# uberkk/ImageCompressionLearnedLiftingandLearnedTreeBasedModels

Measured on AMD Instinct MI355X. Metric: Mpixels/sec (lifting DWT + entropy-model fwd) at 512x512 RGB, higher is better.
Workload: dtype f32 storage, f16x3 arithmetic (3 fp16 MFMA products per fp32 MAC, fp32 accumulate)

## Files before the change

### imagecompressionlearnedliftingandlearnedtreebasedmodels_amd/_lib.py

```python
import ctypes as C
import os

_HERE = os.path.dirname(os.path.abspath(__file__))
LIB_PATH = os.path.join(_HERE, "liblldwt.so")


class LLDWTError(RuntimeError):
    pass


class View(C.Structure):
    _fields_ = [("p", C.c_void_p), ("sz", C.c_int64), ("sy", C.c_int64), ("sx", C.c_int64)]


class LiftOp(C.Structure):
    _fields_ = [("kind", C.c_int32), ("buf_src", C.c_int32), ("buf_din", C.c_int32), ("buf_dout", C.c_int32),
                ("off_src", C.c_int64), ("sz_src", C.c_int64), ("sy_src", C.c_int64), ("sx_src", C.c_int64),
                ("off_din", C.c_int64), ("sz_din", C.c_int64), ("sy_din", C.c_int64), ("sx_din", C.c_int64),
                ("off_dout", C.c_int64), ("sz_dout", C.c_int64), ("sy_dout", C.c_int64), ("sx_dout", C.c_int64),
                ("h", C.c_int32), ("w", C.c_int32), ("vertical", C.c_int32), ("tap", C.c_int32), ("block", C.c_int32),
                ("is_u", C.c_int32), ("sign", C.c_float), ("pad_", C.c_int32), ("saved_off", C.c_int64)]


class ConvDesc(C.Structure):
# ... 39 lines not shown
    "lldwt_train_lift_f16": (_i, []),
    "lldwt_set_precision": (_i, [_i]),
    "lldwt_get_precision": (_i, []),
    "lldwt_set_cdf97_short_levels": (_i, [_i]),
    "lldwt_get_lift_mode": (_i, []),
    "lldwt_pack_pblock": (_i, [_p] * 9 + [_i, _i, _i, _p]),
    "lldwt_pack_pblock_train": (_i, [_p] * 9 + [_i, _i, _i, _p]),
    "lldwt_pack_pblock_seq": (_i, [_p] * 9 + [_i, _i, _i, _p]),
    "lldwt_lift_step_ws_bytes": (_i64, [_i64, _i64, _i64, _i]),
    "lldwt_lift_step": (_i, [View, View, View, _i64, _i64, _i64, _i64, _p, _p, _i, _i, _i, _f, _f, _i, _p, _i64, _p]),
    "lldwt_lifting_ws_bytes": (_i64, [_i64, _i64, _i64, _i]),
    "lldwt_lifting_forward": (_i, [_p, _p, C.POINTER(_p), _i64, _i64, _i64, _i64, _i, _p, _p, _i, _i, _i, _i, _i, _f, _i,
                                   _p, _p, _p, _i64, _p]),
    "lldwt_lifting_inverse": (_i, [_p, C.POINTER(_p), _p, _i64, _i64, _i64, _i64, _i, _p, _p, _i, _i, _i, _i, _f, _i,
                                   _p, _p, _p, _i64, _p]),
    "lldwt_lifting_program": (_i, [C.POINTER(LiftOp), _i, _i64, _i64, _i64, _i, _i, _i, _i, _i, _i, C.POINTER(_i64)]),
    "lldwt_lifting_forward_train": (_i, [_p, _p, C.POINTER(_p), _i64, _i64, _i64, _i64, _i, _p, _p, _i, _i, _i, _i, _i, _f,
                                         _i, _p, _p, _p, _i64, _p, _p]),
    "lldwt_lifting_inverse_train": (_i, [_p, C.POINTER(_p), _p, _i64, _i64, _i64, _i64, _i, _p, _p, _i, _i, _i, _i, _f, _i,
                                         _p, _p, _p, _i64, _p, _p]),
    "lldwt_lift_bwd_pre": (_i, [View, View, _p, _i64, _i64, _i64, _p]),
    "lldwt_lift_bwd_fin": (_i, [_p, _p, _p, View, _i64, _i64, _i64, _i64, _p, _p, _i, _f, _f, _p]),
    "lldwt_lift_step_bwd_ws_bytes": (_i64, [_i64, _i64, _i64, _i]),
    "lldwt_lift_step_bwd": (_i, [View, View, View, _p, _i64, _i64, _i64, _i64, _p, _p, _p, _i64] + [_p] * 8 +
                            [_i, _i, _f, _f, _i, _i, _p, _i64, _p]),
    "lldwt_lift_step_bwd_f16": (_i, [View, View, View, _p, _i64, _i64, _i64, _i64, _p, _p, _p, _i64] + [_p] * 8 +
                                [_i, _i, _f, _f, _i, _i, _p, _i64, _p, _p, _p]),
    "lldwt_bwd_lift_f16": (_i, []),
    "lldwt_pack_pblock_bwd_ws_bytes": (_i64, [_i]),
    "lldwt_pack_pblock_bwd": (_i, [_p, _p, _p, _p, _p, _p, _i64, _i, _i, _i, _p]),
    "lldwt_subband_mlp_bwd_w_ws_bytes": (_i64, [_i64, _i, _i64]),
    "lldwt_subband_mlp_bwd_w": (_i, [_p, _p, _p, _i64, _i64, _i, _i64, _i] + [_p] * 7 + [_p] * 8 + [_p, _i64, _p]),
    "lldwt_subband_mlp_bwd": (_i, [_p] * 9 + [_i64, _i64, _i, _i64, _i] + [_p] * 7 + [_p]),
    "lldwt_subband_mlp": (_i, [_p, _p, _i64, _i64, _i, _i64, _i] + [_p] * 8 + [_i, _p]),
    "lldwt_conv_packed_floats": (_i64, [C.POINTER(ConvDesc)]),
    "lldwt_conv_pack": (_i, [_p, _p, C.POINTER(ConvDesc), _i64, _i, _p]),
    "lldwt_conv2d": (_i, [_p, _p, _p, _p, _p, _p, C.POINTER(ConvDesc), _i64, _i64, _i64, _i64, _p]),
    "lldwt_conv_stack_pair": (_i, [_p, _p, _p, _p, C.POINTER(_p), C.POINTER(_p), C.POINTER(ConvDesc), _i, _i, _p, _p, _i64, _i64, _i64,
                                   _i64, _i64, _i64, _p]),
    "lldwt_conv2d_absmax": (_i, [_p, _p, _p, _p, _p, _p, _p, C.POINTER(ConvDesc), _i64, _i64, _i64, _i64, _p]),
    "lldwt_conv2d_f16out": (_i, [_p, _p, _p, _p, _p, C.POINTER(ConvDesc), _i64, _i64, _i64, _i64, _p]),
    "lldwt_conv3x3_f16in": (_i, [_p, _p, _p, _p, _p, _i, _i, _i, _i64, _i64, _i64, _i64, _p]),
    "lldwt_conv2d_wgrad": (_i, [_p, _p, _p, _p, C.POINTER(ConvDesc), _i64, _i64, _i64, _i64, _f, _i, _p]),
    "lldwt_conv3x3_wgrad_f16x3": (_i, [_p, _p, _p, _p, _p, _p, _p, _i, _i, _i64, _i64, _i64, _i64, _f, _p]),
    "lldwt_conv_f16x3_packed_bytes": (_i64, [_i, _i]),
    "lldwt_plc_shape16": (_i, []),
    "lldwt_plc_winograd": (_i, []),
    "lldwt_plc_fused_pack1_bytes": (_i64, [_i]),
    "lldwt_plc_fused_pack1": (_i, [_p, _p, _p, _i, _i64, _p]),
    "lldwt_plc_fused": (_i, [_p, _p, _p, _p, _p, _i, _i, _i, _i64, _i64, _i64, _i64, _p]),
    "lldwt_conv_f16x3_pack": (_i, [_p, _p, _i, _i, _i64, _p]),
    "lldwt_absmax_slots": (_i, [_p, _i64, _i64, _p, _p]),
    "lldwt_conv3x3_f16x3": (_i, [_p, _p, _p, _p, _p, _i, _i, _i, _i64, _i64, _i64, _i64, _p]),
    "lldwt_act_bwd": (_i, [_p, _p, _p, _i64, _i, _p]),
    "lldwt_downsum2": (_i, [_p, _p, _i64, _i64, _i64, _p]),
    "lldwt_conv2d_direct": (_i, [_p, _p, _p, _p, C.POINTER(ConvDesc), _i64, _i64, _i64, _i64, _p]),
    "lldwt_gdn": (_i, [_p, _p, _p, _p, _i64, _i64, _i, _i64, _i, _f, _p]),
    "lldwt_ew_mul": (_i, [_p, _p, _p, _i64, _f, _p]),
    "lldwt_gdn_apply": (_i, [_p, _p, _p, _i64, _i, _p]),
    "lldwt_gdn_apply_bwd": (_i, [_p, _p, _p, _p, _p, _i64, _i, _p]),
    "lldwt_lower_bound_fwd": (_i, [_p, _p, _i64, _f, _p]),
    "lldwt_lower_bound_bwd": (_i, [_p, _p, _p, _i64, _f, _p]),
    "lldwt_nonneg_param_fwd": (_i, [_p, _p, _i64, _f, _p]),
    "lldwt_nonneg_param_bwd": (_i, [_p, _p, _p, _i64, _f, _p]),
    "lldwt_gauss_rate": (_i, [_p, _p, _p, _p, _p, _p, _i64, _i, _i64, _p]),
    "lldwt_cgp_packed_floats": (_i64, [_i, _i, _i, _i, _i]),
    "lldwt_cgp_pack": (_i, [_p] * 9 + [_i64, _i, _i, _i, _i, _i, _p]),
# ... 89 lines not shown
```

### imagecompressionlearnedliftingandlearnedtreebasedmodels_amd/csrc/ops.hip

```cpp
#include "common.h"
#include <stdlib.h>
#include <string.h>
#include <math.h>

namespace lldwt {

static thread_local char g_err[512] = "";

void set_error(const char* fmt, ...) {
    va_list ap;
    va_start(ap, fmt);
    vsnprintf(g_err, sizeof(g_err), fmt, ap);
    va_end(ap);
}

constexpr float KR = 0.2126f, KG = 0.7152f, KB = 0.0722f;

__global__ void k_rgb_to_ycc(const float* __restrict__ rgb, float* __restrict__ ycc, int64_t B, int64_t hw) {
    const int64_t n = B * hw;
    for (int64_t i = blockIdx.x * (int64_t)blockDim.x + threadIdx.x; i < n; i += (int64_t)gridDim.x * blockDim.x) {
        const int64_t b = i / hw, p = i - b * hw;
        const float r = rgb[(b * 3 + 0) * hw + p], g = rgb[(b * 3 + 1) * hw + p], bl = rgb[(b * 3 + 2) * hw + p];
        const float y = KR * r + KG * g + KB * bl;
        const float cb = 0.5f * (bl - y) / (1.f - KB) + 0.5f;
// ... 144 lines not shown
                                  uint32_t tw, uint32_t ov, uint32_t ny, uint32_t nx, uint32_t y0, uint32_t x0, uint32_t h,
                                  uint32_t w, float inv_ov, float* __restrict__ acc) {
    const uint32_t x = blockIdx.x * blockDim.x + threadIdx.x;
    if (x >= w) return;
    const LapAxis ay = lap_axis(y0 + blockIdx.y, th, ov, ny, inv_ov);
    const LapAxis ax = lap_axis(x0 + x, tw, ov, nx, inv_ov);
    const int32_t qy[2] = {ay.q0, ay.q1}, iy[2] = {ay.i0, ay.i1}, qx[2] = {ax.q0, ax.q1}, ix[2] = {ax.i0, ax.i1};
    const float wy[2] = {ay.w0, ay.w1}, wx[2] = {ax.w0, ax.w1};
    const int64_t hw = (int64_t)th * tw, rhw = (int64_t)h * w, p = (int64_t)blockIdx.y * w + x;
    float a[3];
    bool any = false;
#pragma unroll
    for (int c = 0; c < 3; ++c) a[c] = acc[c * rhw + p];
#pragma unroll
    for (int u = 0; u < 2; ++u) {
#pragma unroll
        for (int v = 0; v < 2; ++v) {
            if (qy[u] < 0 || qx[v] < 0) continue;
            const int32_t j = slots[(int64_t)qy[u] * nx + qx[v]];
            if (j < 0 || j >= n) continue;
            const float wt = __fmul_rn(wy[u], wx[v]);
            const int64_t q = (int64_t)iy[u] * tw + ix[v];
#pragma unroll
            for (int c = 0; c < 3; ++c) a[c] = __fadd_rn(a[c], __fmul_rn(wt, ycc[(c * n + j) * hw + q]));
            any = true;
        }
    }
    if (!any) return;
#pragma unroll
    for (int c = 0; c < 3; ++c) acc[c * rhw + p] = a[c];
}

typedef float floatx4m __attribute__((ext_vector_type(4)));
__global__ __launch_bounds__(256) void k_subband_mlp_mfma(const float* __restrict__ x, float* __restrict__ y, int batch, int C,
                                                          int64_t hw, const float* __restrict__ w0,
                                                          const float* __restrict__ b0, const float* __restrict__ w1,
                                                          const float* __restrict__ b1, const float* __restrict__ w2,
                                                          const float* __restrict__ b2, const float* __restrict__ w3,
                                                          const float* __restrict__ b3, int transposed) {
    constexpr int HD = 32;
    const int c = blockIdx.y;
    const int64_t z = blockIdx.z;
    const int plane = (int)(z / batch);
    const int64_t pc = (int64_t)plane * C + c;
    const int lane = threadIdx.x & 63, wave = threadIdx.x >> 6;
    const int col = lane & 15, kk = lane >> 4;
    float A1[2][8], A2[2][8], w0b[8], b0b[8], b1d[8], b2d[8], w3d[8];
#pragma unroll
    for (int m = 0; m < 2; ++m)
#pragma unroll
        for (int q = 0; q < 8; ++q) {
            const int oc = m * 16 + col, ic = (q >> 2) * 16 + 4 * kk + (q & 3);
            const int64_t src = transposed ? (pc * HD + ic) * HD + oc : (pc * HD + oc) * HD + ic;
            A1[m][q] = w1[src];
            A2[m][q] = w2[src];
        }
#pragma unroll
    for (int q = 0; q < 8; ++q) {
        const int ch = (q >> 2) * 16 + 4 * kk + (q & 3);
        w0b[q] = w0[pc * HD + ch];
        b0b[q] = b0[pc * HD + ch];
        b1d[q] = b1[pc * HD + ch];
        b2d[q] = b2[pc * HD + ch];
        w3d[q] = w3[pc * HD + ch];
    }
    const float bb3 = b3[pc];
    const float* xp = x + (z * C + c) * hw;
    float* yp = y + (z * C + c) * hw;
    for (int64_t i0 = ((int64_t)blockIdx.x * 4 + wave) * 64; i0 < hw; i0 += (int64_t)gridDim.x * 256) {
        float xv[4];
#pragma unroll
        for (int n = 0; n < 4; ++n) {
            const int64_t i = i0 + n * 16 + col;
            xv[n] = xp[i < hw ? i : 0];
        }
        float h[4][8];
#pragma unroll
        for (int n = 0; n < 4; ++n)
#pragma unroll
            for (int q = 0; q < 8; ++q) h[n][q] = fast_tanh(fmaf(w0b[q], xv[n], b0b[q]));
#pragma unroll
        for (int layer = 0; layer < 2; ++layer) {
            floatx4m acc[2][4];
#pragma unroll
            for (int m = 0; m < 2; ++m)
#pragma unroll
                for (int n = 0; n < 4; ++n) {
                    const float* bd = layer == 0 ? b1d : b2d;
                    acc[m][n] = floatx4m{bd[m * 4 + 0], bd[m * 4 + 1], bd[m * 4 + 2], bd[m * 4 + 3]};
                }
#pragma unroll
            for (int q = 0; q < 8; ++q)
#pragma unroll
                for (int m = 0; m < 2; ++m)
#pragma unroll
                    for (int n = 0; n < 4; ++n)
                        acc[m][n] = __builtin_amdgcn_mfma_f32_16x16x4f32(layer == 0 ? A1[m][q] : A2[m][q], h[n][q], acc[m][n],
                                                                         0, 0, 0);
#pragma unroll
            for (int n = 0; n < 4; ++n)
#pragma unroll
                for (int m = 0; m < 2; ++m)
#pragma unroll
                    for (int r = 0; r < 4; ++r) h[n][m * 4 + r] = fast_tanh(acc[m][n][r]);
        }
#pragma unroll
        for (int n = 0; n < 4; ++n) {
            float o = 0.f;
#pragma unroll
            for (int q = 0; q < 8; ++q) o = fmaf(w3d[q], h[n][q], o);
            o += __shfl_xor(o, 16, 64);
            o += __shfl_xor(o, 32, 64);
            const int64_t i = i0 + n * 16 + col;
            if (kk == 0 && i < hw) yp[i] = o + bb3;
        }
    }
}

__global__ __launch_bounds__(256) void k_subband_mlp_bwd(const float* __restrict__ x, const float* __restrict__ gy,
                                                         float* __restrict__ gx, float* __restrict__ h0o,
                                                         float* __restrict__ h1o, float* __restrict__ h2o,
                                                         float* __restrict__ d0o, float* __restrict__ d1o,
                                                         float* __restrict__ d2o, int batch, int C, int64_t hw,
                                                         const float* __restrict__ w0, const float* __restrict__ b0,
                                                         const float* __restrict__ w1, const float* __restrict__ b1,
                                                         const float* __restrict__ w2, const float* __restrict__ b2,
                                                         const float* __restrict__ w3) {
    constexpr int HD = 32, NC = 2;
    const int c = blockIdx.y;
    const int64_t z = blockIdx.z;
    const int plane = (int)(z / batch);
    const int64_t pc = (int64_t)plane * C + c;
    const int lane = threadIdx.x & 63, wave = threadIdx.x >> 6;
    const int col = lane & 15, kk = lane >> 4;
    float A1[2][8], A2[2][8], A1T[2][8], A2T[2][8], w0b[8], b0b[8], b1d[8], b2d[8], w3d[8];
#pragma unroll
    for (int m = 0; m < 2; ++m)
#pragma unroll
        for (int q = 0; q < 8; ++q) {
            const int row = m * 16 + col, ch = (q >> 2) * 16 + 4 * kk + (q & 3);
            A1[m][q] = w1[(pc * HD + row) * HD + ch];
            A2[m][q] = w2[(pc * HD + row) * HD + ch];
            A1T[m][q] = w1[(pc * HD + ch) * HD + row];
            A2T[m][q] = w2[(pc * HD + ch) * HD + row];
        }
#pragma unroll
    for (int q = 0; q < 8; ++q) {
        const int ch = (q >> 2) * 16 + 4 * kk + (q & 3);
        w0b[q] = w0[pc * HD + ch];
        b0b[q] = b0[pc * HD + ch];
// ... 975 lines not shown
    return check_launch("u8hwc_to_ycc_tiles_lapped");
}
extern "C" int lldwt_ycc_tiles_blend(const float* ycc, const int32_t* slots, int64_t nslots, int64_t n, int64_t H, int64_t W,
                                     int64_t th, int64_t tw, int64_t ov, int64_t ny, int64_t nx, int64_t y0, int64_t x0,
                                     int64_t h, int64_t w, float* acc, void* stream) {
    LLDWT_REQUIRE(ycc && slots && acc, "ycc_tiles_blend: null pointer");
    if (const int rc = lapped_grid_ok("ycc_tiles_blend", H, W, th, tw, ov, ny, nx)) return rc;
    LLDWT_REQUIRE(ny * nx < (1ll << 31) && nslots == ny * nx, "ycc_tiles_blend: the slot table holds %lld entries, the grid "
                  "has %lld tiles", (long long)nslots, (long long)(ny * nx));
    LLDWT_REQUIRE(n > 0 && n <= nslots, "ycc_tiles_blend: %lld tiles in the group, the grid has %lld", (long long)n,
                  (long long)nslots);
    LLDWT_REQUIRE(y0 >= 0 && x0 >= 0 && h > 0 && w > 0 && y0 + h <= H && x0 + w <= W,
                  "ycc_tiles_blend: region (%lld, %lld, %lld, %lld) outside the %lld x %lld image", (long long)y0,
                  (long long)x0, (long long)h, (long long)w, (long long)H, (long long)W);
    LLDWT_REQUIRE(h <= 65535, "ycc_tiles_blend: grid too large");
    hipLaunchKernelGGL(k_ycc_tiles_blend, dim3((unsigned)cdiv(w, 256), (unsigned)h), dim3(256), 0, (hipStream_t)stream, ycc,
                       slots, n, (uint32_t)th, (uint32_t)tw, (uint32_t)ov, (uint32_t)ny, (uint32_t)nx, (uint32_t)y0,
                       (uint32_t)x0, (uint32_t)h, (uint32_t)w, 1.0f / (float)ov, acc);
    return check_launch("ycc_tiles_blend");
}
extern "C" int lldwt_u8hwc_to_ycc_pad(const uint8_t* src, float* ycc, int64_t B, int64_t H, int64_t W, int64_t Hp, int64_t Wp,
                                      void* stream) {
    LLDWT_REQUIRE(src && ycc && B > 0 && H > 0 && W > 0 && Hp >= H && Wp >= W, "u8hwc_to_ycc_pad: bad arguments");
    LLDWT_REQUIRE(B <= 65535 && Hp <= 65535 && Wp <= (1ll << 30), "u8hwc_to_ycc_pad: grid too large");
    return lldwt_u8hwc_to_ycc_tiles(src, ycc, B, H, W, Hp, Wp, 1, 1, 0, B, stream);
}
extern "C" int lldwt_ycc_to_u8hwc_crop(const float* ycc, uint8_t* dst, int64_t B, int64_t H, int64_t W, int64_t Hp, int64_t Wp,
                                       void* stream) {
    LLDWT_REQUIRE(ycc && dst && B > 0 && H > 0 && W > 0 && Hp >= H && Wp >= W, "ycc_to_u8hwc_crop: bad arguments");
    LLDWT_REQUIRE(B <= 65535 && H <= 65535 && W <= (1ll << 30), "ycc_to_u8hwc_crop: grid too large");
    return lldwt_ycc_tiles_to_u8hwc(ycc, nullptr, 0, B, B, H, W, Hp, Wp, 1, 1, 0, 0, H, W, dst, stream);
}

extern "C" int lldwt_subband_mlp(const float* x, float* y, int64_t planes, int64_t batch, int C, int64_t hw, int Hd,
                                 const float* w0, const float* b0, const float* w1, const float* b1, const float* w2,
                                 const float* b2, const float* w3, const float* b3, int transposed, void* stream) {
    LLDWT_REQUIRE(x && y && w0 && b0 && w1 && b1 && w2 && b2 && w3 && b3, "subband_mlp: null pointer");
    LLDWT_REQUIRE(planes > 0 && batch > 0 && C > 0 && hw > 0, "subband_mlp: bad dims");
    LLDWT_REQUIRE(Hd == 32, "subband_mlp: hidden width %d unsupported (reference uses H=32, lifting_dwt_nets.py:98)", Hd);
    LLDWT_REQUIRE(planes * batch <= 65535 && C <= 65535, "subband_mlp: grid too large");
    int64_t gx = cdiv(hw, 256);
    if (gx > 1024) gx = 1024;
    dim3 grid((unsigned)gx, (unsigned)C, (unsigned)(planes * batch));
    hipLaunchKernelGGL(k_subband_mlp_mfma, grid, dim3(256), 0, (hipStream_t)stream, x, y, (int)batch, C, hw, w0, b0, w1, b1,
                       w2, b2, w3, b3, transposed);
    return check_launch("subband_mlp");
}

extern "C" int lldwt_subband_mlp_bwd(const float* x, const float* gy, float* gx, float* h0, float* h1, float* h2, float* d0,
                                     float* d1, float* d2, int64_t planes, int64_t batch, int C, int64_t hw, int Hd,
                                     const float* w0, const float* b0, const float* w1, const float* b1, const float* w2,
                                     const float* b2, const float* w3, void* stream) {
    LLDWT_REQUIRE(x && gy && gx && h0 && h1 && h2 && d0 && d1 && d2 && w0 && b0 && w1 && b1 && w2 && b2 && w3,
                  "subband_mlp_bwd: null pointer");
    LLDWT_REQUIRE(planes > 0 && batch > 0 && C > 0 && hw > 0, "subband_mlp_bwd: bad dims");
    LLDWT_REQUIRE(Hd == 32, "subband_mlp_bwd: hidden width %d unsupported (reference uses H=32, lifting_dwt_nets.py:98)", Hd);
    LLDWT_REQUIRE(planes * batch <= 65535 && C <= 65535, "subband_mlp_bwd: grid too large");
    int64_t gxn = cdiv(hw, 128);
    if (gxn > 1024) gxn = 1024;
    dim3 grid((unsigned)gxn, (unsigned)C, (unsigned)(planes * batch));
    hipLaunchKernelGGL(k_subband_mlp_bwd, grid, dim3(256), 0, (hipStream_t)stream, x, gy, gx, h0, h1, h2, d0, d1, d2, (int)batch,
                       C, hw, w0, b0, w1, b1, w2, b2, w3);
    return check_launch("subband_mlp_bwd");
}

static inline int64_t mlpw_slices(int64_t planes, int C, int64_t hw) {
    int64_t s = (int64_t)lldwt_num_cus() * 2 / (planes * C);
    const int64_t most = cdiv(hw, 128);
    s = s > most ? most : s;
    return s < 1 ? 1 : s;
}
extern "C" int64_t lldwt_subband_mlp_bwd_w_ws_bytes(int64_t planes, int C, int64_t hw) {
    return (int64_t)sizeof(float) * planes * C * mlpw_slices(planes, C, hw) * 4 * MLPW_ROW;
}
extern "C" int lldwt_subband_mlp_bwd_w(const float* x, const float* gy, float* gx, int64_t planes, int64_t batch, int C, int64_t hw,
                                       int Hd, const float* w0, const float* b0, const float* w1, const float* b1,
                                       const float* w2, const float* b2, const float* w3, float* dw0, float* db0, float* dw1,
                                       float* db1, float* dw2, float* db2, float* dw3, float* db3, void* ws, int64_t ws_bytes,
                                       void* stream) {
    LLDWT_REQUIRE(x && gy && gx && w0 && b0 && w1 && b1 && w2 && b2 && w3 && dw0 && db0 && dw1 && db1 && dw2 && db2 && dw3 && db3 &&
                  ws, "subband_mlp_bwd_w: null pointer");
// ... 264 lines not shown
```

### imagecompressionlearnedliftingandlearnedtreebasedmodels_amd/graphs/layers/lifting_dwt_nets.py

```python
import torch
from torch import nn

from ... import ops
from ...packed_cache import PackedOwnerMixin, cached
from .P_block_v2 import P_block_v2
from .gdn import GDN
from .wavelet_forward_v2 import wavelet_forward_v2
from .wavelet_inverse_v2 import wavelet_inverse_v2

lifting_coeff = [-1.586134342059924, -0.052980118572961, 0.882911075530934, 0.443506852043971, 0.869864451624781,
                 1.149604398860241]


def get_cdf97_filters(oned_or_twod="2D"):
    lp = torch.tensor([0.0, 0.037828455507264, -0.023849465019557, -0.110624404418437, 0.377402855612831,
                       0.852698679008894, 0.377402855612831, -0.110624404418437, -0.023849465019557,
                       0.037828455507264], dtype=torch.double)
    hp = torch.tensor([0.0, -0.064538882628697, 0.040689417609164, 0.418092273221617, -0.788485616405583,
                       0.418092273221617, 0.040689417609164, -0.064538882628697, 0.0, 0.0], dtype=torch.double)
    slp = torch.tensor([0.0, -0.064538882628697, -0.040689417609164, 0.418092273221617, 0.788485616405583,
                        0.418092273221617, -0.040689417609164, -0.064538882628697, 0.0, 0.0], dtype=torch.double)
    shp = torch.tensor([0.0, -0.037828455507264, -0.023849465019557, 0.110624404418437, 0.377402855612831,
                        -0.852698679008894, 0.377402855612831, 0.110624404418437, -0.023849465019557,
                        -0.037828455507264], dtype=torch.double)
# ... 32 lines not shown


class SubbandAutoEncoderBerk(PackedOwnerMixin, nn.Module):

    def __init__(self, in_ch):
        super().__init__()
        self._init_packed_owner()
        iC, H, K, P = in_ch, 64, 3, 1
        self.in_ch = iC
        self.ae_down = nn.Sequential(
            nn.Conv2d(iC, iC * H // 2, K, padding=P), GDN(iC * H // 2), nn.Conv2d(iC * H // 2, iC * H, K, padding=P),
            GDN(iC * H), nn.Conv2d(iC * H, iC * H // 2, K, padding=P), GDN(iC * H // 2),
            nn.Conv2d(iC * H // 2, iC, K, padding=P))
        self.ae_up = nn.Sequential(
            nn.ConvTranspose2d(iC, iC * H // 2, K, padding=P), GDN(iC * H // 2, inverse=True),
            nn.ConvTranspose2d(iC * H // 2, iC * H, K, padding=P), GDN(iC * H, inverse=True),
            nn.ConvTranspose2d(iC * H, iC * H // 2, K, padding=P), GDN(iC * H // 2, inverse=True),
            nn.ConvTranspose2d(iC * H // 2, iC, K, padding=P))

    def encode(self, x):
        return ae_planes([self], x[None].contiguous(), False)[0]

    def decode(self, y_hat):
        return ae_planes([self], y_hat[None].contiguous(), True)[0]


def ae_planes(aes, x, decode):
    seq = [(a.ae_up if decode else a.ae_down) for a in aes]
    tag = ("ae", decode)
    own = aes[0]
    if isinstance(aes[0], SubbandAutoEncoder):
        convs = [[s[n] for s in seq] for n in (0, 2, 4, 6)]
        srcs = [p for layer in convs for m in layer for p in (m.weight, m.bias)]
        ws = cached(own, tag, srcs, lambda: [t for layer in convs for t in (
            _stack(layer, lambda m: m.weight).flatten(1), _stack(layer, lambda m: m.bias))])
        return ops.subband_mlp(x, *ws, transposed=decode, hidden=aes[0].H)
    t = x
    for n in (0, 2, 4, 6):
        layer = [s[n] for s in seq]
        w, b = cached(own, tag + (n,), [p for m in layer for p in (m.weight, m.bias)],
                          lambda: (_stack(layer, lambda m: m.weight), _stack(layer, lambda m: m.bias)))
        t = ops.conv2d(t, w, b, 3, transposed=decode)
        if n != 6:
            g = [s[n + 1] for s in seq]
            beta, gamma = cached(own, tag + (n, "g"), [p for m in g for p in (m.beta, m.gamma)],
                                     lambda: (_stack(g, lambda m: m.beta), _stack(g, lambda m: m.gamma)))
            t = ops.gdn(t, beta, gamma, inverse=decode, beta_min=g[0].beta_min)
    return t


class DWTPytorchWaveletsLayer(PackedOwnerMixin, nn.Module):

    def __init__(self, config):
        super().__init__()
        self._init_packed_owner()
        self.dwtlevels = config.dwtlevels
        self.clrch = config.clrch
        self.Yl_ae = SubbandAutoEncoder(in_ch=1 * config.clrch)
        self.Yh_ae = nn.ModuleList([SubbandAutoEncoder(in_ch=3 * config.clrch) for _ in range(self.dwtlevels)])

    def encode(self, x):
        xe, xo = encode_planes([self], x[None].contiguous())
        return xe[0], [t[0] for t in xo]

    def decode(self, out_xe, out_xo_list):
        return decode_planes([self], out_xe[None].contiguous(), [t[None].contiguous() for t in out_xo_list])[0]


class LiftingBasedNeuralWaveletv4(PackedOwnerMixin, nn.Module):
# ... 177 lines not shown
```

### imagecompressionlearnedliftingandlearnedtreebasedmodels_amd/ops.py

```python
import ctypes as C
import os

import torch

from . import _lib
from ._lib import (ACT_LRELU, ACT_NONE, ACT_RELU, ACT_TANH, EPI_LRELU_BWD, EPI_NONE, EPI_TANH_BWD, ConvDesc, View,
                   check)

_ws = {}


def _env_choice(name, default, allowed):
    v = os.environ.get(name, default)
    if v not in allowed:
        names = " or ".join(a if a.isdigit() else repr(a) for a in allowed)
        raise _lib.LLDWTError("%s must be %s (got %r)" % (name, names, v))
    return v


def plc_mode():
    return _env_choice("LLDWT_PLC_MODE", "f16x3", ("f32", "f16x3"))


def train_lift_f16():
# ... 333 lines not shown
    check(_lib.load().lldwt_set_cdf97_short_levels(1 if periodic else 0), "lldwt_set_cdf97_short_levels")


def cdf97_forward(x, levels, adj=False):
    lib = _lib.load()
    P, B, Cc, H, W = x.shape
    Z = P * B * Cc
    dev = x.device
    ll = torch.empty(P, B, Cc, H >> levels, W >> levels, device=dev, dtype=torch.float32)
    yh = [torch.empty(P, B, Cc, 3, H >> (i + 1), W >> (i + 1), device=dev, dtype=torch.float32) for i in range(levels)]
    nb = lib.lldwt_cdf97_ws_bytes(Z, H, W)
    ws = workspace(nb, dev)
    check(lib.lldwt_cdf97_forward(_chk(x, "x"), _chk(ll), _ptr_array(yh), Z, H, W, levels, int(bool(adj)),
                                     C.c_void_p(ws.data_ptr()), nb, _stream()), "cdf97_forward")
    return ll, yh


def cdf97_inverse(ll, yh, adj=False):
    lib = _lib.load()
    levels = len(yh)
    P, B, Cc, hl, wl = ll.shape
    H, W = hl << levels, wl << levels
    Z = P * B * Cc
    x = torch.empty(P, B, Cc, H, W, device=ll.device, dtype=torch.float32)
    for t in yh:
        _chk(t, "yh")
    nb = lib.lldwt_cdf97_ws_bytes(Z, H, W)
    ws = workspace(nb, ll.device)
    check(lib.lldwt_cdf97_inverse(_chk(ll, "ll"), _ptr_array(yh), _chk(x), Z, H, W, levels, int(bool(adj)),
                                     C.c_void_p(ws.data_ptr()), nb, _stream()), "cdf97_inverse")
    return x


def subband_mlp(x, w0, b0, w1, b1, w2, b2, w3, b3, transposed=False, hidden=32):
    lib = _lib.load()
    P, B, Cc, h, w = x.shape
    y = torch.empty_like(x)
    check(lib.lldwt_subband_mlp(_chk(x, "x"), _chk(y), P, B, Cc, h * w, hidden, _chk(w0), _chk(b0), _chk(w1), _chk(b1),
                                _chk(w2), _chk(b2), _chk(w3), _chk(b3), int(bool(transposed)), _stream()), "subband_mlp")
    return y


def subband_mlp_bwd(x, gy, w0, b0, w1, b1, w2, b2, w3, hidden=32):
    P, B, Cc, h, w = x.shape
    gx = torch.empty_like(x)
    hs = [torch.empty(P, B, Cc * hidden, h, w, device=x.device, dtype=torch.float32) for _ in range(6)]
    check(_lib.load().lldwt_subband_mlp_bwd(_chk(x, "x"), _chk(gy, "gy"), _chk(gx), *[_chk(t) for t in hs], P, B, Cc, h * w,
                                            hidden, _chk(w0), _chk(b0), _chk(w1), _chk(b1), _chk(w2), _chk(b2), _chk(w3),
                                            _stream()), "subband_mlp_bwd")
    return gx, hs[:3], hs[3:]


def subband_mlp_bwd_w(x, gy, w0, b0, w1, b1, w2, b2, w3, hidden=32):
    lib = _lib.load()
    P, B, Cc, h, w = x.shape
    gx = torch.empty_like(x)
    shapes = [(P, Cc * hidden, 1, 1, 1), (P, Cc * hidden), (P, Cc * hidden, hidden, 1, 1), (P, Cc * hidden),
              (P, Cc * hidden, hidden, 1, 1), (P, Cc * hidden), (P, Cc, hidden, 1, 1), (P, Cc)]
    g = [torch.empty(s, device=x.device, dtype=torch.float32) for s in shapes]
    nb = lib.lldwt_subband_mlp_bwd_w_ws_bytes(P, Cc, h * w)
    ws = workspace(nb, x.device)
    check(lib.lldwt_subband_mlp_bwd_w(_chk(x, "x"), _chk(gy, "gy"), _chk(gx), P, B, Cc, h * w, hidden, _chk(w0), _chk(b0),
                                      _chk(w1), _chk(b1), _chk(w2), _chk(b2), _chk(w3), *[_chk(t) for t in g],
                                      C.c_void_p(ws.data_ptr()), nb, _stream()), "subband_mlp_bwd_w")
    return gx, g


def conv_desc(cin, cout, K, groups=1, act=ACT_NONE, upsample2=False, transposed=False, tap_mask=None, oc_block=None,
              oc_stride=0, oc_off=0, ytot=None, ic_block=0, ic_stride=0, ic_off=0, xtot=0, epi=0):
    return ConvDesc(cin, cout, K, groups, act, int(bool(upsample2)), int(bool(transposed)),
                    (1 << (K * K)) - 1 if tap_mask is None else int(tap_mask), cout if oc_block is None else oc_block,
                    oc_stride, oc_off, cout if ytot is None else ytot, ic_block, ic_stride, ic_off, xtot, epi)
# ... 801 lines not shown
```

### include/lldwt.h

```cpp
#ifndef LLDWT_H
#define LLDWT_H

#include <stdint.h>

#ifdef __cplusplus
extern "C" {
#endif

#define LLDWT_OK 0
#define LLDWT_EINVAL (-1)
#define LLDWT_EHIP (-2)
#define LLDWT_EWS (-3)

#define LLDWT_ACT_NONE 0
#define LLDWT_ACT_TANH 1
#define LLDWT_ACT_LRELU 2
#define LLDWT_ACT_RELU 3

const char* lldwt_last_error(void);
int lldwt_version(void);
int lldwt_device_ok(void);

typedef struct lldwt_view {
    float* p;
// ... 70 lines not shown
                          int block_offset, int inverse, int scale, int C, int64_t* saved_floats);
int lldwt_lifting_forward_train(const float* x, float* ll, float* const* yh, int64_t planes, int64_t batch, int64_t H,
                                int64_t W, int levels, const float* taps, const float* packed, int nblocks,
                                int block_offset, int different, int C, int K, float res_weight, int linear,
                                const float* scale_nh, const float* scale_nl, void* ws, int64_t ws_bytes, float* saved,
                                void* stream);
int lldwt_lifting_inverse_train(const float* ll, const float* const* yh, float* x, int64_t planes, int64_t batch,
                                int64_t H, int64_t W, int levels, const float* taps, const float* packed, int nblocks,
                                int block_offset, int C, int K, float res_weight, int linear, const float* scale_nh,
                                const float* scale_nl, void* ws, int64_t ws_bytes, float* saved, void* stream);
int lldwt_lift_bwd_pre(lldwt_view g_dst_out, lldwt_view g_dst_in, float* g, int64_t Z, int64_t h, int64_t w, void* stream);
int lldwt_lift_bwd_fin(const float* g, const float* dsk, const float* srcv, lldwt_view g_src, int64_t Z, int64_t batch,
                       int64_t h, int64_t w, const float* taps, float* dtaps, int vertical, float sign, float res_weight,
                       void* stream);

int64_t lldwt_lift_step_bwd_ws_bytes(int64_t Z, int64_t h, int64_t w, int C);
int lldwt_lift_step_bwd(lldwt_view g_dst_out, lldwt_view g_dst_in, lldwt_view g_src, const float* saved_step,
                        int64_t planes, int64_t batch, int64_t h, int64_t w, const float* taps, float* dtaps,
                        const float* packed, int64_t packed_plane_stride, float* dw1, float* db1, float* dw2, float* db2,
                        float* dw3, float* db3, float* dw4, float* db4, int C, int K, float res_weight, float sign,
                        int vertical, int linear, void* ws, int64_t ws_bytes, void* stream);

int lldwt_bwd_lift_f16(void);
int64_t lldwt_pack_pblock_bwd_ws_bytes(int planes);
int lldwt_pack_pblock_bwd(const float* w1, const float* w2, const float* w3, const float* w4, float* packed, void* ws,
                          int64_t ws_bytes, int planes, int C, int K, void* stream);
int lldwt_lift_step_bwd_f16(lldwt_view g_dst_out, lldwt_view g_dst_in, lldwt_view g_src, const float* saved_step,
                            int64_t planes, int64_t batch, int64_t h, int64_t w, const float* taps, float* dtaps,
                            const float* packed, int64_t packed_plane_stride, float* dw1, float* db1, float* dw2, float* db2,
                            float* dw3, float* db3, float* dw4, float* db4, int C, int K, float res_weight, float sign,
                            int vertical, int linear, void* ws, int64_t ws_bytes, const float* packed_bwd,
                            const float* taps_id, void* stream);

int lldwt_subband_mlp(const float* x, float* y, int64_t planes, int64_t batch, int C, int64_t hw, int Hd,
                      const float* w0, const float* b0, const float* w1, const float* b1, const float* w2,
                      const float* b2, const float* w3, const float* b3, int transposed, void* stream);
int lldwt_subband_mlp_bwd(const float* x, const float* gy, float* gx, float* h0, float* h1, float* h2, float* d0, float* d1,
                          float* d2, int64_t planes, int64_t batch, int C, int64_t hw, int Hd, const float* w0,
                          const float* b0, const float* w1, const float* b1, const float* w2, const float* b2,
                          const float* w3, void* stream);
int64_t lldwt_subband_mlp_bwd_w_ws_bytes(int64_t planes, int C, int64_t hw);
int lldwt_subband_mlp_bwd_w(const float* x, const float* gy, float* gx, int64_t planes, int64_t batch, int C, int64_t hw, int Hd,
                            const float* w0, const float* b0, const float* w1, const float* b1, const float* w2,
                            const float* b2, const float* w3, float* dw0, float* db0, float* dw1, float* db1, float* dw2,
                            float* db2, float* dw3, float* db3, void* ws, int64_t ws_bytes, void* stream);

typedef struct lldwt_conv_desc {
    int cin, cout, K, groups;
    int act;
    int upsample2;
    int transposed;
    uint32_t tap_mask;
    int oc_block, oc_stride, oc_off, ytot;
    int ic_block, ic_stride, ic_off, xtot;
    int epi;
} lldwt_conv_desc;
#define LLDWT_EPI_NONE 0
#define LLDWT_EPI_TANH_BWD 1
#define LLDWT_EPI_LRELU_BWD 2
int64_t lldwt_conv_packed_floats(const lldwt_conv_desc* d);
int lldwt_conv_pack(const float* w, float* packed, const lldwt_conv_desc* d, int64_t planes, int swap_hw, void* stream);
int lldwt_conv2d(const float* x, float* y, const float* packed, const float* bias, const float* residual,
                 const float* aux, const lldwt_conv_desc* d, int64_t planes, int64_t batch, int64_t h, int64_t w_,
                 void* stream);
int lldwt_conv_stack_pair(const float* xa, const float* xb, float* ya, float* yb, const float* const* packed,
                          const float* const* bias, const lldwt_conv_desc* descs, int nlayers, int groups_a, float* ws0,
                          float* ws1, int64_t ws0_floats, int64_t ws1_floats, int64_t planes, int64_t batch, int64_t h, int64_t w_, void* stream);
int lldwt_conv2d_absmax(const float* x, float* y, const float* packed, const float* bias, const float* residual,
                        const float* aux, float* absmax_slots, const lldwt_conv_desc* d, int64_t planes, int64_t batch,
// ... 191 lines not shown
```

Before: 197.2.

## Move subband MLP to split-fp16 MFMA with prepacked cached weights

```diff
diff --git a/imagecompressionlearnedliftingandlearnedtreebasedmodels_amd/_lib.py b/imagecompressionlearnedliftingandlearnedtreebasedmodels_amd/_lib.py
--- a/imagecompressionlearnedliftingandlearnedtreebasedmodels_amd/_lib.py
+++ b/imagecompressionlearnedliftingandlearnedtreebasedmodels_amd/_lib.py
@@ -95,7 +95,9 @@
     "lldwt_subband_mlp_bwd_w_ws_bytes": (_i64, [_i64, _i, _i64]),
     "lldwt_subband_mlp_bwd_w": (_i, [_p, _p, _p, _i64, _i64, _i, _i64, _i] + [_p] * 7 + [_p] * 8 + [_p, _i64, _p]),
     "lldwt_subband_mlp_bwd": (_i, [_p] * 9 + [_i64, _i64, _i, _i64, _i] + [_p] * 7 + [_p]),
-    "lldwt_subband_mlp": (_i, [_p, _p, _i64, _i64, _i, _i64, _i] + [_p] * 8 + [_i, _p]),
+    "lldwt_subband_mlp_packed_bytes": (_i64, [_i64, _i]),
+    "lldwt_subband_mlp_pack": (_i, [_p] * 8 + [_i64, _i, _i, _i, _p, _i64, _p]),
+    "lldwt_subband_mlp": (_i, [_p, _p, _i64, _i64, _i, _i64, _i, _p, _i64, _p]),
     "lldwt_conv_packed_floats": (_i64, [C.POINTER(ConvDesc)]),
     "lldwt_conv_pack": (_i, [_p, _p, C.POINTER(ConvDesc), _i64, _i, _p]),
     "lldwt_conv2d": (_i, [_p, _p, _p, _p, _p, _p, C.POINTER(ConvDesc), _i64, _i64, _i64, _i64, _p]),
diff --git a/imagecompressionlearnedliftingandlearnedtreebasedmodels_amd/csrc/ops.hip b/imagecompressionlearnedliftingandlearnedtreebasedmodels_amd/csrc/ops.hip
--- a/imagecompressionlearnedliftingandlearnedtreebasedmodels_amd/csrc/ops.hip
+++ b/imagecompressionlearnedliftingandlearnedtreebasedmodels_amd/csrc/ops.hip
@@ -200,90 +200,6 @@
 }
 
 typedef float floatx4m __attribute__((ext_vector_type(4)));
-__global__ __launch_bounds__(256) void k_subband_mlp_mfma(const float* __restrict__ x, float* __restrict__ y, int batch, int C,
-                                                          int64_t hw, const float* __restrict__ w0,
-                                                          const float* __restrict__ b0, const float* __restrict__ w1,
-                                                          const float* __restrict__ b1, const float* __restrict__ w2,
-                                                          const float* __restrict__ b2, const float* __restrict__ w3,
-                                                          const float* __restrict__ b3, int transposed) {
-    constexpr int HD = 32;
-    const int c = blockIdx.y;
-    const int64_t z = blockIdx.z;
-    const int plane = (int)(z / batch);
-    const int64_t pc = (int64_t)plane * C + c;
-    const int lane = threadIdx.x & 63, wave = threadIdx.x >> 6;
-    const int col = lane & 15, kk = lane >> 4;
-    float A1[2][8], A2[2][8], w0b[8], b0b[8], b1d[8], b2d[8], w3d[8];
-#pragma unroll
-    for (int m = 0; m < 2; ++m)
-#pragma unroll
-        for (int q = 0; q < 8; ++q) {
-            const int oc = m * 16 + col, ic = (q >> 2) * 16 + 4 * kk + (q & 3);
-            const int64_t src = transposed ? (pc * HD + ic) * HD + oc : (pc * HD + oc) * HD + ic;
-            A1[m][q] = w1[src];
-            A2[m][q] = w2[src];
-        }
-#pragma unroll
-    for (int q = 0; q < 8; ++q) {
-        const int ch = (q >> 2) * 16 + 4 * kk + (q & 3);
-        w0b[q] = w0[pc * HD + ch];
-        b0b[q] = b0[pc * HD + ch];
-        b1d[q] = b1[pc * HD + ch];
-        b2d[q] = b2[pc * HD + ch];
-        w3d[q] = w3[pc * HD + ch];
-    }
-    const float bb3 = b3[pc];
-    const float* xp = x + (z * C + c) * hw;
-    float* yp = y + (z * C + c) * hw;
-    for (int64_t i0 = ((int64_t)blockIdx.x * 4 + wave) * 64; i0 < hw; i0 += (int64_t)gridDim.x * 256) {
-        float xv[4];
-#pragma unroll
-        for (int n = 0; n < 4; ++n) {
-            const int64_t i = i0 + n * 16 + col;
-            xv[n] = xp[i < hw ? i : 0];
-        }
-        float h[4][8];
-#pragma unroll
-        for (int n = 0; n < 4; ++n)
-#pragma unroll
-            for (int q = 0; q < 8; ++q) h[n][q] = fast_tanh(fmaf(w0b[q], xv[n], b0b[q]));
-#pragma unroll
-        for (int layer = 0; layer < 2; ++layer) {
-            floatx4m acc[2][4];
-#pragma unroll
-            for (int m = 0; m < 2; ++m)
-#pragma unroll
-                for (int n = 0; n < 4; ++n) {
-                    const float* bd = layer == 0 ? b1d : b2d;
-                    acc[m][n] = floatx4m{bd[m * 4 + 0], bd[m * 4 + 1], bd[m * 4 + 2], bd[m * 4 + 3]};
-                }
-#pragma unroll
-            for (int q = 0; q < 8; ++q)
-#pragma unroll
-                for (int m = 0; m < 2; ++m)
-#pragma unroll
-                    for (int n = 0; n < 4; ++n)
-                        acc[m][n] = __builtin_amdgcn_mfma_f32_16x16x4f32(layer == 0 ? A1[m][q] : A2[m][q], h[n][q], acc[m][n],
-                                                                         0, 0, 0);
-#pragma unroll
-            for (int n = 0; n < 4; ++n)
-#pragma unroll
-                for (int m = 0; m < 2; ++m)
-#pragma unroll
-                    for (int r = 0; r < 4; ++r) h[n][m * 4 + r] = fast_tanh(acc[m][n][r]);
-        }
-#pragma unroll
-        for (int n = 0; n < 4; ++n) {
-            float o = 0.f;
-#pragma unroll
-            for (int q = 0; q < 8; ++q) o = fmaf(w3d[q], h[n][q], o);
-            o += __shfl_xor(o, 16, 64);
-            o += __shfl_xor(o, 32, 64);
-            const int64_t i = i0 + n * 16 + col;
-            if (kk == 0 && i < hw) yp[i] = o + bb3;
-        }
-    }
-}
 
 __global__ __launch_bounds__(256) void k_subband_mlp_bwd(const float* __restrict__ x, const float* __restrict__ gy,
                                                          float* __restrict__ gx, float* __restrict__ h0o,
@@ -1325,21 +1241,6 @@
     return lldwt_ycc_tiles_to_u8hwc(ycc, nullptr, 0, B, B, H, W, Hp, Wp, 1, 1, 0, 0, H, W, dst, stream);
 }
 
-extern "C" int lldwt_subband_mlp(const float* x, float* y, int64_t planes, int64_t batch, int C, int64_t hw, int Hd,
-                                 const float* w0, const float* b0, const float* w1, const float* b1, const float* w2,
-                                 const float* b2, const float* w3, const float* b3, int transposed, void* stream) {
-    LLDWT_REQUIRE(x && y && w0 && b0 && w1 && b1 && w2 && b2 && w3 && b3, "subband_mlp: null pointer");
-    LLDWT_REQUIRE(planes > 0 && batch > 0 && C > 0 && hw > 0, "subband_mlp: bad dims");
-    LLDWT_REQUIRE(Hd == 32, "subband_mlp: hidden width %d unsupported (reference uses H=32, lifting_dwt_nets.py:98)", Hd);
-    LLDWT_REQUIRE(planes * batch <= 65535 && C <= 65535, "subband_mlp: grid too large");
-    int64_t gx = cdiv(hw, 256);
-    if (gx > 1024) gx = 1024;
-    dim3 grid((unsigned)gx, (unsigned)C, (unsigned)(planes * batch));
-    hipLaunchKernelGGL(k_subband_mlp_mfma, grid, dim3(256), 0, (hipStream_t)stream, x, y, (int)batch, C, hw, w0, b0, w1, b1,
-                       w2, b2, w3, b3, transposed);
-    return check_launch("subband_mlp");
-}
-
 extern "C" int lldwt_subband_mlp_bwd(const float* x, const float* gy, float* gx, float* h0, float* h1, float* h2, float* d0,
                                      float* d1, float* d2, int64_t planes, int64_t batch, int C, int64_t hw, int Hd,
                                      const float* w0, const float* b0, const float* w1, const float* b1, const float* w2,
diff --git a/imagecompressionlearnedliftingandlearnedtreebasedmodels_amd/csrc/subband_mlp_f16.hip b/imagecompressionlearnedliftingandlearnedtreebasedmodels_amd/csrc/subband_mlp_f16.hip
--- /dev/null
+++ b/imagecompressionlearnedliftingandlearnedtreebasedmodels_amd/csrc/subband_mlp_f16.hip
@@ -0,0 +1,200 @@
+#include "split_f16.h"
+
+namespace lldwt {
+namespace {
+
+constexpr int SMLP_HD = 32;
+constexpr int SMLP_A_FLOATS = 2048, SMLP_V_FLOATS = 160, SMLP_S_FLOATS = 8;
+constexpr int SMLP_PC_FLOATS = SMLP_A_FLOATS + SMLP_V_FLOATS + SMLP_S_FLOATS;
+constexpr float SMLP_ACT_SCALE = 16384.f;
+
+__device__ __forceinline__ int smlp_channel(int kk, int j) { return (j >> 2) * 16 + 4 * kk + (j & 3); }
+
+__global__ __launch_bounds__(64) void k_subband_mlp_pack(const float* __restrict__ w0, const float* __restrict__ b0,
+                                                         const float* __restrict__ w1, const float* __restrict__ b1,
+                                                         const float* __restrict__ w2, const float* __restrict__ b2,
+                                                         const float* __restrict__ w3, const float* __restrict__ b3,
+                                                         int transposed, float* __restrict__ pack) {
+    constexpr int HD = SMLP_HD;
+    const int64_t pc = blockIdx.x;
+    const int lane = threadIdx.x, col = lane & 15, kk = lane >> 4;
+    float* out = pack + pc * SMLP_PC_FLOATS;
+    float scale[2];
+#pragma unroll
+    for (int layer = 0; layer < 2; ++layer) {
+        const float* W = (layer == 0 ? w1 : w2) + pc * HD * HD;
+        float amax = 0.f;
+        for (int i = lane; i < HD * HD; i += 64) amax = fmaxf(amax, fabsf(W[i]));
+#pragma unroll
+        for (int o = 32; o > 0; o >>= 1) amax = fmaxf(amax, __shfl_xor(amax, o, 64));
+        const float s = fminf(fmaxf(pow2_scale<15>(amax), 0x1p-113f), 0x1p112f);
+        scale[layer] = s;
+#pragma unroll
+        for (int m = 0; m < 2; ++m) {
+            float v[8];
+#pragma unroll
+            for (int j = 0; j < 8; ++j) {
+                const int oc = m * 16 + col, ic = smlp_channel(kk, j);
+                v[j] = W[transposed ? ic * HD + oc : oc * HD + ic] * s;
+            }
+            h8_t hi, lo;
+            split8v(v, hi, lo);
+            h8_t* frag = reinterpret_cast<h8_t*>(out) + ((layer * 2 + m) * 2) * 64 + lane;
+            frag[0] = hi;
+            frag[64] = lo;
+        }
+    }
+    if (lane < 32) {
+        const int k4 = lane >> 3, j = lane & 7, ch = smlp_channel(k4, j);
+        const float* src[5] = {w0, b0, b1, b2, w3};
+#pragma unroll
+        for (int a = 0; a < 5; ++a) out[SMLP_A_FLOATS + a * 32 + lane] = src[a][pc * HD + ch];
+    }
+    if (lane < 8) {
+        float v = 0.f;
+        if (lane < 2) v = scale[lane];
+        else if (lane < 4) v = (1.f / scale[lane - 2]) * (1.f / SMLP_ACT_SCALE);
+        else if (lane == 4) v = b3[pc];
+        out[SMLP_A_FLOATS + SMLP_V_FLOATS + lane] = v;
+    }
+}
+
+__device__ __forceinline__ float tanh_act(float x) {
+    const float e = __builtin_amdgcn_exp2f(fabsf(x) * 2.88539008177792681472f);
+    const float t = __builtin_fmaf(-2.f * SMLP_ACT_SCALE, __builtin_amdgcn_rcpf(e + 1.f), SMLP_ACT_SCALE);
+    return copysignf(t, x);
+}
+
+__global__ __launch_bounds__(256, 2) void k_subband_mlp_f16(const float* __restrict__ x, float* __restrict__ y, int batch, int C,
+                                                         int64_t hw, int64_t nblk, const float* __restrict__ pack) {
+    const int64_t pc = blockIdx.y;
+    const int plane = (int)(pc / C), c = (int)(pc % C);
+    const int lane = threadIdx.x & 63, wave = threadIdx.x >> 6;
+    const int col = lane & 15, kk = lane >> 4;
+    const float* pk = pack + pc * SMLP_PC_FLOATS;
+    h8_t A[2][2][2];
+#pragma unroll
+    for (int f = 0; f < 8; ++f) A[f >> 2][(f >> 1) & 1][f & 1] = reinterpret_cast<const h8_t*>(pk)[f * 64 + lane];
+    float vec[5][8];
+#pragma unroll
+    for (int a = 0; a < 5; ++a)
+#pragma unroll
+        for (int hlf = 0; hlf < 2; ++hlf) {
+            const floatx4 v = reinterpret_cast<const floatx4*>(pk + SMLP_A_FLOATS)[(a * 4 + kk) * 2 + hlf];
+#pragma unroll
+            for (int r = 0; r < 4; ++r) vec[a][hlf * 4 + r] = v[r];
+        }
+    const floatx4 sc = reinterpret_cast<const floatx4*>(pk + SMLP_A_FLOATS + SMLP_V_FLOATS)[0];
+    const float inv[2] = {sc[2], sc[3]};
+    const float bb3 = pk[SMLP_A_FLOATS + SMLP_V_FLOATS + 4];
+#pragma unroll
+    for (int q = 0; q < 8; ++q) vec[4][q] *= 1.f / SMLP_ACT_SCALE;
+
+    const int64_t stride = (int64_t)gridDim.x * 4, first = (int64_t)blockIdx.x * 4 + __builtin_amdgcn_readfirstlane(wave);
+    const int64_t simg = stride / nblk, sblk = stride - simg * nblk;
+    int64_t img = first / nblk, blk = first - img * nblk;
+    for (; img < batch; img += simg, blk += sblk) {
+        if (blk >= nblk) {
+            blk -= nblk;
+            if (++img >= batch) break;
+        }
+        const int64_t i0 = blk * 64;
+        const int64_t base = (((int64_t)plane * batch + img) * C + c) * hw;
+        const float* xp = x + base;
+        float* yp = y + base;
+        float xv[4];
+#pragma unroll
+        for (int n = 0; n < 4; ++n) {
+            const int64_t i = i0 + n * 16 + col;
+            xv[n] = xp[i < hw ? i : 0];
+        }
+        float h[4][8];
+#pragma unroll
+        for (int n = 0; n < 4; ++n)
+#pragma unroll
+            for (int q = 0; q < 8; ++q) h[n][q] = tanh_act(fmaf(vec[0][q], xv[n], vec[1][q]));
+#pragma unroll
+        for (int layer = 0; layer < 2; ++layer) {
+            f4_t acc[2][4];
+#pragma unroll
+            for (int n = 0; n < 4; ++n) {
+                h8_t hi, lo;
+                split8v(h[n], hi, lo);
+#pragma unroll
+                for (int m = 0; m < 2; ++m) {
+                    f4_t a = {0.f, 0.f, 0.f, 0.f};
+                    a = mma16<0>(A[layer][m][1], hi, a);
+                    a = mma16<0>(A[layer][m][0], lo, a);
+                    acc[m][n] = mma16<0>(A[layer][m][0], hi, a);
+                }
+            }
+#pragma unroll
+            for (int n = 0; n < 4; ++n)
+#pragma unroll
+                for (int m = 0; m < 2; ++m)
+#pragma unroll
+                    for (int r = 0; r < 4; ++r)
+                        h[n][m * 4 + r] = tanh_act(fmaf(acc[m][n][r], inv[layer], vec[2 + layer][m * 4 + r]));
+        }
+        float o[4];
+#pragma unroll
+        for (int n = 0; n < 4; ++n) {
+            float s = 0.f;
+#pragma unroll
+            for (int q = 0; q < 8; ++q) s = fmaf(vec[4][q], h[n][q], s);
+            s += __shfl_xor(s, 16, 64);
+            s += __shfl_xor(s, 32, 64);
+            o[n] = s;
+        }
+        const float ov = kk == 0 ? o[0] : kk == 1 ? o[1] : kk == 2 ? o[2] : o[3];
+        const int64_t i = i0 + lane;
+        if (i < hw) yp[i] = ov + bb3;
+    }
+}
+
+}
+}
+
+using namespace lldwt;
+
+extern "C" int64_t lldwt_subband_mlp_packed_bytes(int64_t planes, int C) {
+    if (planes <= 0 || C <= 0) return 0;
+    return planes * C * SMLP_PC_FLOATS * (int64_t)sizeof(float);
+}
+
+extern "C" int lldwt_subband_mlp_pack(const float* w0, const float* b0, const float* w1, const float* b1, const float* w2,
+                                      const float* b2, const float* w3, const float* b3, int64_t planes, int C, int Hd,
+                                      int transposed, void* pack, int64_t pack_bytes, void* stream) {
+    LLDWT_REQUIRE(w0 && b0 && w1 && b1 && w2 && b2 && w3 && b3 && pack, "subband_mlp_pack: null pointer");
+    LLDWT_REQUIRE(planes > 0 && C > 0 && planes * C <= 0x7fffffff, "subband_mlp_pack: bad dims");
+    LLDWT_REQUIRE(Hd == SMLP_HD, "subband_mlp_pack: hidden width %d unsupported (reference uses H=32, lifting_dwt_nets.py:98)", Hd);
+    LLDWT_REQUIRE(((uintptr_t)pack & 15) == 0, "subband_mlp_pack: pack must be 16-byte aligned");
+    LLDWT_REQUIRE(pack_bytes >= lldwt_subband_mlp_packed_bytes(planes, C), "subband_mlp_pack: pack of %ld bytes, %ld needed",
+                  (long)pack_bytes, (long)lldwt_subband_mlp_packed_bytes(planes, C));
+    hipLaunchKernelGGL(k_subband_mlp_pack, dim3((unsigned)(planes * C)), dim3(64), 0, (hipStream_t)stream, w0, b0, w1, b1, w2, b2,
+                       w3, b3, transposed, (float*)pack);
+    return check_launch("subband_mlp_pack");
+}
+
+extern "C" int lldwt_subband_mlp(const float* x, float* y, int64_t planes, int64_t batch, int C, int64_t hw, int Hd,
+                                 const void* pack, int64_t pack_bytes, void* stream) {
+    LLDWT_REQUIRE(x && y && pack, "subband_mlp: null pointer");
+    LLDWT_REQUIRE(planes > 0 && batch > 0 && C > 0 && hw > 0, "subband_mlp: bad dims");
+    LLDWT_REQUIRE(Hd == SMLP_HD, "subband_mlp: hidden width %d unsupported (reference uses H=32, lifting_dwt_nets.py:98)", Hd);
+    LLDWT_REQUIRE(planes * C <= 65535 && batch <= 0x7fffffff, "subband_mlp: grid too large");
+    LLDWT_REQUIRE(((uintptr_t)pack & 15) == 0, "subband_mlp: pack must be 16-byte aligned");
+    LLDWT_REQUIRE(pack_bytes >= lldwt_subband_mlp_packed_bytes(planes, C), "subband_mlp: pack of %ld bytes, %ld needed",
+                  (long)pack_bytes, (long)lldwt_subband_mlp_packed_bytes(planes, C));
+    static int occ = 0;
+    if (occ <= 0 && (hipOccupancyMaxActiveBlocksPerMultiprocessor(&occ, k_subband_mlp_f16, 256, 0) != hipSuccess || occ <= 0)) {
+        (void)hipGetLastError();
+        occ = 2;
+    }
+    const int64_t nblk = cdiv(hw, 64), pairs = planes * C;
+    int64_t g = (int64_t)lldwt_num_cus() * occ / pairs;
+    if (g < 1) g = 1;
+    if (g > cdiv(nblk * batch, 4)) g = cdiv(nblk * batch, 4);
+    hipLaunchKernelGGL(k_subband_mlp_f16, dim3((unsigned)g, (unsigned)pairs), dim3(256), 0, (hipStream_t)stream, x, y, (int)batch,
+                       C, hw, nblk, (const float*)pack);
+    return check_launch("subband_mlp");
+}
diff --git a/imagecompressionlearnedliftingandlearnedtreebasedmodels_amd/graphs/layers/lifting_dwt_nets.py b/imagecompressionlearnedliftingandlearnedtreebasedmodels_amd/graphs/layers/lifting_dwt_nets.py
--- a/imagecompressionlearnedliftingandlearnedtreebasedmodels_amd/graphs/layers/lifting_dwt_nets.py
+++ b/imagecompressionlearnedliftingandlearnedtreebasedmodels_amd/graphs/layers/lifting_dwt_nets.py
@@ -88,9 +88,11 @@
     if isinstance(aes[0], SubbandAutoEncoder):
         convs = [[s[n] for s in seq] for n in (0, 2, 4, 6)]
         srcs = [p for layer in convs for m in layer for p in (m.weight, m.bias)]
-        ws = cached(own, tag, srcs, lambda: [t for layer in convs for t in (
-            _stack(layer, lambda m: m.weight).flatten(1), _stack(layer, lambda m: m.bias))])
-        return ops.subband_mlp(x, *ws, transposed=decode, hidden=aes[0].H)
+        def build():
+            ws = [t for layer in convs for t in (_stack(layer, lambda m: m.weight).flatten(1), _stack(layer, lambda m: m.bias))]
+            return ws, ops.subband_mlp_pack(*ws, transposed=decode, hidden=aes[0].H)
+        ws, pack = cached(own, tag, srcs, build)
+        return ops.subband_mlp(x, *ws, transposed=decode, hidden=aes[0].H, pack=pack)
     t = x
     for n in (0, 2, 4, 6):
         layer = [s[n] for s in seq]
diff --git a/imagecompressionlearnedliftingandlearnedtreebasedmodels_amd/ops.py b/imagecompressionlearnedliftingandlearnedtreebasedmodels_amd/ops.py
--- a/imagecompressionlearnedliftingandlearnedtreebasedmodels_amd/ops.py
+++ b/imagecompressionlearnedliftingandlearnedtreebasedmodels_amd/ops.py
@@ -389,12 +389,25 @@
     return x
 
 
-def subband_mlp(x, w0, b0, w1, b1, w2, b2, w3, b3, transposed=False, hidden=32):
+def subband_mlp_pack(w0, b0, w1, b1, w2, b2, w3, b3, transposed=False, hidden=32):
+    lib = _lib.load()
+    P, Cc = b3.shape
+    nb = lib.lldwt_subband_mlp_packed_bytes(P, Cc)
+    pack = torch.empty(nb, dtype=torch.uint8, device=w0.device)
+    check(lib.lldwt_subband_mlp_pack(_chk(w0), _chk(b0), _chk(w1), _chk(b1), _chk(w2), _chk(b2), _chk(w3), _chk(b3), P, Cc,
+                                     hidden, int(bool(transposed)), C.c_void_p(pack.data_ptr()), nb, _stream()),
+          "subband_mlp_pack")
+    return pack
+
+
+def subband_mlp(x, w0, b0, w1, b1, w2, b2, w3, b3, transposed=False, hidden=32, pack=None):
     lib = _lib.load()
     P, B, Cc, h, w = x.shape
+    if pack is None:
+        pack = subband_mlp_pack(w0, b0, w1, b1, w2, b2, w3, b3, transposed=transposed, hidden=hidden)
     y = torch.empty_like(x)
-    check(lib.lldwt_subband_mlp(_chk(x, "x"), _chk(y), P, B, Cc, h * w, hidden, _chk(w0), _chk(b0), _chk(w1), _chk(b1),
-                                _chk(w2), _chk(b2), _chk(w3), _chk(b3), int(bool(transposed)), _stream()), "subband_mlp")
+    check(lib.lldwt_subband_mlp(_chk(x, "x"), _chk(y), P, B, Cc, h * w, hidden, C.c_void_p(pack.data_ptr()), pack.numel(),
+                                _stream()), "subband_mlp")
     return y
 
 
diff --git a/include/lldwt.h b/include/lldwt.h
--- a/include/lldwt.h
+++ b/include/lldwt.h
@@ -126,9 +126,12 @@
                             int vertical, int linear, void* ws, int64_t ws_bytes, const float* packed_bwd,
                             const float* taps_id, void* stream);
 
-int lldwt_subband_mlp(const float* x, float* y, int64_t planes, int64_t batch, int C, int64_t hw, int Hd,
-                      const float* w0, const float* b0, const float* w1, const float* b1, const float* w2,
-                      const float* b2, const float* w3, const float* b3, int transposed, void* stream);
+int64_t lldwt_subband_mlp_packed_bytes(int64_t planes, int C);
+int lldwt_subband_mlp_pack(const float* w0, const float* b0, const float* w1, const float* b1, const float* w2,
+                           const float* b2, const float* w3, const float* b3, int64_t planes, int C, int Hd, int transposed,
+                           void* pack, int64_t pack_bytes, void* stream);
+int lldwt_subband_mlp(const float* x, float* y, int64_t planes, int64_t batch, int C, int64_t hw, int Hd, const void* pack,
+                      int64_t pack_bytes, void* stream);
 int lldwt_subband_mlp_bwd(const float* x, const float* gy, float* gx, float* h0, float* h1, float* h2, float* d0, float* d1,
                           float* d2, int64_t planes, int64_t batch, int C, int64_t hw, int Hd, const float* w0,
                           const float* b0, const float* w1, const float* b1, const float* w2, const float* b2,
```

Result: faster. 200.7, median of 6 (+1.8%).
